# alexandrainst/coral

Measured on AMD Instinct MI355X. Metric: audio-seconds/sec (CTC finetune step: fwd+bwd+allreduce+clip+AdamW), wav2vec2-large, 10 s utterances, higher is better.
Workload: dtype bf16; 1 GPU; wav2vec2-large (XLS-R shape d=1920 L=48 ffn=7680) CTC finetune, 8 x 10 s per GPU, SpecAugment on, activation_dropout 0.1, layerdrop 0 (multi-GPU rule), fp32 master + AdamW + clip 1.0; global_batch=8, frames_per_utt=499, parallelism=dp1

## Files before the change

coral_amd/csrc/ctc.hip:

```cpp
#include "common.h"

#define NEG_INF (-__builtin_inff())

__device__ __forceinline__ float log_add3(float a, float b, float c) {
  const float m = fmaxf(a, fmaxf(b, c));
  if (m == NEG_INF) return NEG_INF;
  return m + __logf(__expf(a - m) + __expf(b - m) + __expf(c - m));
}
__device__ __forceinline__ float log_add2(float a, float b) {
  const float m = fmaxf(a, b);
  if (m == NEG_INF) return NEG_INF;
  return m + __logf(__expf(a - m) + __expf(b - m));
}

struct CtcWs {
  float* lp;
  float* alpha;
  float* beta;
};

__device__ __host__ inline int64_t align256(int64_t x) { return (x + 255) & ~(int64_t)255; }

extern "C" int64_t ca_ctc_workspace_bytes(int32_t B, int32_t T, int32_t Lmax) {
  const int64_t S = 2 * (int64_t)Lmax + 1;
  return align256((int64_t)B * T * 256 * 4) + 2 * align256((int64_t)B * T * S * 4) + align256((int64_t)B * 4);
}

#define CTC_MAXS 1025

__global__ __launch_bounds__(256) void ctc_logsoftmax_kernel(const float* __restrict__ logits, float* __restrict__ lp,
                                                             int64_t frames, int V, int64_t ldv) {
  const int lane = threadIdx.x & 63;
  const int64_t f = (int64_t)blockIdx.x * 4 + (threadIdx.x >> 6);
  if (f >= frames) return;
  const float* l = logits + f * ldv;
  float x[4];
  float mx = NEG_INF;
#pragma unroll
  for (int j = 0; j < 4; ++j) {
    const int v = lane + 64 * j;
    x[j] = v < V ? l[v] : NEG_INF;
    mx = fmaxf(mx, x[j]);
  }
  mx = wave_max(mx);
  float s = 0.f;
#pragma unroll
  for (int j = 0; j < 4; ++j) s += (lane + 64 * j) < V ? __expf(x[j] - mx) : 0.f;
  s = wave_sum(s);
  const float lse = mx + __logf(s);
#pragma unroll
  for (int j = 0; j < 4; ++j)
    if (lane + 64 * j < V) lp[f * V + lane + 64 * j] = x[j] - lse;
}

__global__ __launch_bounds__(512) void ctc_kernel(const int32_t* __restrict__ labels,
                                                  const int32_t* __restrict__ in_len,
                                                  float* __restrict__ nll_out,
                                                  float* __restrict__ raw_nll, const float* __restrict__ lp,
                                                  float* alpha, float* beta, int T, int V,
                                                  int Lmax, int Smax, int blank, int zero_inf, int lp_in_lds) {
  __shared__ int ext[CTC_MAXS];
  __shared__ float rowa[2][CTC_MAXS];
  __shared__ float rowb[2][CTC_MAXS];
  __shared__ int sh_L;
  __shared__ float sh_nll;
  extern __shared__ float lds_lp[];
  const int b = blockIdx.x;
  const int tid = threadIdx.x;
  const int lane = tid & 63, wave = tid >> 6;
  const float* lpb = lp + (int64_t)b * T * V;
  if (lp_in_lds)
    for (int i = tid; i < T * V; i += 512) lds_lp[i] = lpb[i];
  float* ab = alpha + (int64_t)b * T * Smax;
  float* bb = beta + (int64_t)b * T * Smax;
  int Tin = in_len ? in_len[b] : T;
  if (Tin > T) Tin = T;
  if (Tin < 0) Tin = 0;

  if (tid == 0) {
    int L = 0;
    for (int i = 0; i < Lmax; ++i) {
      const int c = labels[(int64_t)b * Lmax + i];
      if (c >= 0) {
        ext[2 * L] = blank;
        ext[2 * L + 1] = c;
        ++L;
      }
    }
    ext[2 * L] = blank;
    sh_L = L;
  }
  __syncthreads();
  const int L = sh_L;
  const int S = 2 * L + 1;
  const bool is_alpha = tid < 256;
  const int st = tid & 255;

  if (S <= 256) {
    if (wave < 2 && Tin > 0) {
      const bool fwd = wave == 0;
      float* tab = fwd ? ab : bb;
      int c[4];
      bool skip[4], valid[4];
      float a[4];
#pragma unroll
      for (int j = 0; j < 4; ++j) {
        const int s = 4 * lane + j;
        valid[j] = s < S;
        c[j] = valid[j] ? ext[s] : blank;
        const int s2 = fwd ? s - 2 : s + 2;
        skip[j] = valid[j] && s2 >= 0 && s2 < S && c[j] != blank && ext[s2] != c[j];
      }
      const int t0 = fwd ? 0 : Tin - 1;
      auto lpv = [&](int tt, int cc) -> float { return lp_in_lds ? lds_lp[tt * V + cc] : lpb[(int64_t)tt * V + cc]; };
#pragma unroll
      for (int j = 0; j < 4; ++j) {
        const int s = 4 * lane + j;
        const bool init = fwd ? (s == 0 || s == 1) : (s == S - 1 || s == S - 2);
        a[j] = (valid[j] && init) ? lpv(t0, c[j]) : NEG_INF;
        if (valid[j]) tab[(int64_t)t0 * Smax + s] = a[j];
      }
      float nx[4];
      if (Tin > 1) {
#pragma unroll
        for (int j = 0; j < 4; ++j) nx[j] = lpv(fwd ? 1 : Tin - 2, c[j]);
      }
      for (int step = 1; step < Tin; ++step) {
        const int tt = fwd ? step : Tin - 1 - step;
        float cur[4];
#pragma unroll
        for (int j = 0; j < 4; ++j) cur[j] = nx[j];
        if (step + 1 < Tin) {
#pragma unroll
          for (int j = 0; j < 4; ++j) nx[j] = lpv(fwd ? step + 1 : Tin - 2 - step, c[j]);
        }
        float n1, n2;
        if (fwd) {
          n1 = __shfl_up(a[3], 1, 64);
          n2 = __shfl_up(a[2], 1, 64);
          if (lane == 0) n1 = n2 = NEG_INF;
        } else {
          n1 = __shfl_down(a[0], 1, 64);
          n2 = __shfl_down(a[1], 1, 64);
          if (lane == 63) n1 = n2 = NEG_INF;
        }
        float na[4];
        if (fwd) {
          na[0] = log_add3(a[0], n1, skip[0] ? n2 : NEG_INF);
          na[1] = log_add3(a[1], a[0], skip[1] ? n1 : NEG_INF);
          na[2] = log_add3(a[2], a[1], skip[2] ? a[0] : NEG_INF);
          na[3] = log_add3(a[3], a[2], skip[3] ? a[1] : NEG_INF);
        } else {
          na[3] = log_add3(a[3], n1, skip[3] ? n2 : NEG_INF);
          na[2] = log_add3(a[2], a[3], skip[2] ? n1 : NEG_INF);
          na[1] = log_add3(a[1], a[2], skip[1] ? a[3] : NEG_INF);
          na[0] = log_add3(a[0], a[1], skip[0] ? a[2] : NEG_INF);
        }
#pragma unroll
        for (int j = 0; j < 4; ++j) {
          a[j] = valid[j] ? na[j] + cur[j] : NEG_INF;
          if (valid[j]) tab[(int64_t)tt * Smax + 4 * lane + j] = a[j];
        }
      }
      if (fwd) {
#pragma unroll
        for (int j = 0; j < 4; ++j)
          if (valid[j]) rowa[(Tin - 1) & 1][4 * lane + j] = a[j];
      }
    }
    __syncthreads();
  } else {
    if (Tin > 0) {
      if (is_alpha) {
        for (int s = st; s < S; s += 256) {
          float a = NEG_INF;
          if (s == 0) a = lpb[blank];
          else if (s == 1) a = lpb[ext[1]];
          rowa[0][s] = a;
          ab[s] = a;
        }
      } else {
        const float* lpt = lpb + (int64_t)(Tin - 1) * V;
        for (int s = st; s < S; s += 256) {
          float v = NEG_INF;
          if (s == S - 1) v = lpt[blank];
          else if (s == S - 2) v = lpt[ext[S - 2]];
          rowb[0][s] = v;
          bb[(int64_t)(Tin - 1) * Smax + s] = v;
        }
      }
    }
    __syncthreads();
    for (int step = 1; step < Tin; ++step) {
      const int cur = step & 1, prv = cur ^ 1;
      if (is_alpha) {
        const int t = step;
        const float* lpt = lpb + (int64_t)t * V;
        for (int s = st; s < S; s += 256) {
          const int c = ext[s];
          const float a0 = rowa[prv][s];
          const float a1 = s >= 1 ? rowa[prv][s - 1] : NEG_INF;
          const float a2 = (s >= 2 && c != blank && ext[s - 2] != c) ? rowa[prv][s - 2] : NEG_INF;
          const float a = log_add3(a0, a1, a2) + lpt[c];
          rowa[cur][s] = a;
          ab[(int64_t)t * Smax + s] = a;
        }
      } else {
        const int t = Tin - 1 - step;
        const float* lpt = lpb + (int64_t)t * V;
        for (int s = st; s < S; s += 256) {
          const int c = ext[s];
          const float b0 = rowb[prv][s];
          const float b1 = s + 1 < S ? rowb[prv][s + 1] : NEG_INF;
          const float b2 =
              (s + 2 < S && c != blank && ext[s + 2] != c) ? rowb[prv][s + 2] : NEG_INF;
          const float v = log_add3(b0, b1, b2) + lpt[c];
          rowb[cur][s] = v;
          bb[(int64_t)t * Smax + s] = v;
        }
      }
      __syncthreads();
    }
  }
  if (tid == 0) {
    float nll;
    if (Tin <= 0) {
      nll = __builtin_inff();
    } else {
      const int lastrow = (Tin - 1) & 1;
      const float l1 = rowa[lastrow][S - 1];
      const float l2 = S >= 2 ? rowa[lastrow][S - 2] : NEG_INF;
      nll = -log_add2(l1, l2);
    }
    sh_nll = nll;
  }
  __syncthreads();
  float nll = sh_nll;
  const bool infeasible = !(nll < __builtin_inff());
  if (tid == 0) {
    nll_out[b] = (infeasible && zero_inf) ? 0.f : nll;
    raw_nll[b] = nll;
  }
}

__global__ __launch_bounds__(512) void ctc_grad_kernel(const int32_t* __restrict__ labels,
                                                       const int32_t* __restrict__ in_len,
                                                       const float* __restrict__ raw_nll, float* __restrict__ grad,
                                                       const float* __restrict__ gscale, const float* __restrict__ lp,
                                                       const float* __restrict__ alpha, const float* __restrict__ beta,
                                                       int T, int V, int64_t ldv, int Lmax, int Smax, int blank) {
  __shared__ int ext[CTC_MAXS];
  __shared__ float vm[8][256], vs[8][256];
  __shared__ int sh_L;
  const int b = blockIdx.y;
  const int tid = threadIdx.x;
  const int lane = tid & 63, wave = tid >> 6;
  if (tid == 0) {
    int L = 0;
    for (int i = 0; i < Lmax; ++i) {
      const int c = labels[(int64_t)b * Lmax + i];
      if (c >= 0) {
        ext[2 * L] = blank;
        ext[2 * L + 1] = c;
        ++L;
      }
    }
    ext[2 * L] = blank;
    sh_L = L;
  }
  __syncthreads();
  const int S = 2 * sh_L + 1;
  int Tin = in_len ? in_len[b] : T;
  if (Tin > T) Tin = T;
  if (Tin < 0) Tin = 0;
  const float nll = raw_nll[b];
  const bool infeasible = !(nll < __builtin_inff());
  const float gs = gscale ? gscale[b] : 1.f;
  const int t = blockIdx.x * 8 + wave;
  if (t >= T) return;
  float* g = grad + ((int64_t)b * T + t) * ldv;
  if (t >= Tin || infeasible) {
    for (int v = lane; v < (int)ldv; v += 64) g[v] = 0.f;
    return;
  }
  float* vmax = vm[wave];
  float* vsum = vs[wave];
  for (int v = lane; v < V; v += 64) {
    vmax[v] = NEG_INF;
    vsum[v] = 0.f;
  }
  const float* at = alpha + ((int64_t)b * T + t) * Smax;
  const float* bt = beta + ((int64_t)b * T + t) * Smax;
  for (int s = lane; s < S; s += 64) {
    const float val = at[s] + bt[s];
    if (val > NEG_INF)
      __builtin_amdgcn_ds_fmaxf((__attribute__((address_space(3))) float*)&vmax[ext[s]], val, 0, 0, false);
  }
  asm volatile("s_waitcnt lgkmcnt(0)" ::: "memory");
  for (int s = lane; s < S; s += 64) {
    const float val = at[s] + bt[s];
    if (val > NEG_INF) {
      const int cc = ext[s];
      __builtin_amdgcn_ds_faddf((__attribute__((address_space(3))) float*)&vsum[cc], __expf(val - vmax[cc]), 0, 0, false);
    }
  }
  asm volatile("s_waitcnt lgkmcnt(0)" ::: "memory");
  const float* lpt = lp + ((int64_t)b * T + t) * V;
  for (int v = lane; v < (int)ldv; v += 64) {
    if (v < V) {
      const float l = lpt[v];
      const float res = vsum[v] > 0.f ? vmax[v] + __logf(vsum[v]) : NEG_INF;
      g[v] = (__expf(l) - __expf(res + nll - l)) * gs;
    } else {
      g[v] = 0.f;
    }
  }
}

extern "C" int ca_ctc_loss_fwd_bwd(const float* logits, const int32_t* labels,
                                   const int32_t* in_len, float* nll, float* grad,
                                   const float* gscale, void* ws, int32_t B, int32_t T, int32_t V,
                                   int64_t ldv, int32_t Lmax, int32_t blank, int32_t zero_infinity,
                                   void* stream) {
  CA_CHECK_ARG(logits && labels && nll && ws, "ca_ctc_loss_fwd_bwd: null pointer");
  CA_CHECK_ARG(B > 0 && T > 0 && V > 0 && V <= 256 && ldv >= V && Lmax >= 0,
               "ca_ctc_loss_fwd_bwd: bad shape (V must be <= 256)");
  CA_CHECK_ARG(2 * Lmax + 1 <= CTC_MAXS, "ca_ctc_loss_fwd_bwd: Lmax %d too long (max %d)", Lmax,
               (CTC_MAXS - 1) / 2);
  CA_CHECK_ARG(blank >= 0 && blank < V, "ca_ctc_loss_fwd_bwd: bad blank");
  const int Smax = 2 * Lmax + 1;
  char* w = (char*)ws;
  float* lp = (float*)w;
  w += align256((int64_t)B * T * 256 * 4);
  float* alpha = (float*)w;
  w += align256((int64_t)B * T * Smax * 4);
  float* beta = (float*)w;
  w += align256((int64_t)B * T * Smax * 4);
  float* raw_nll = (float*)w;
  hipStream_t s = (hipStream_t)stream;
  const int64_t frames = (int64_t)B * T;
  hipLaunchKernelGGL(ctc_logsoftmax_kernel, dim3((unsigned)((frames + 3) / 4)), dim3(256), 0, s, logits, lp, frames, V,
                     ldv);
  const size_t lp_bytes = (size_t)T * V * sizeof(float);
  const int lp_in_lds = lp_bytes <= 120 * 1024 ? 1 : 0;
  static bool attr = false;
  if (!attr) {
    hipFuncSetAttribute((const void*)ctc_kernel, hipFuncAttributeMaxDynamicSharedMemorySize, 120 * 1024);
    attr = true;
  }
  hipLaunchKernelGGL(ctc_kernel, dim3(B), dim3(512), lp_in_lds ? lp_bytes : 0, s, labels, in_len, nll, raw_nll, lp, alpha,
                     beta, T, V, Lmax, Smax, blank, zero_infinity, lp_in_lds);
  if (grad)
    hipLaunchKernelGGL(ctc_grad_kernel, dim3((unsigned)((T + 7) / 8), B), dim3(512), 0, s, labels, in_len, raw_nll, grad,
                       gscale, lp, alpha, beta, T, V, ldv, Lmax, Smax, blank);
  CA_CHECK_LAUNCH("ca_ctc_loss_fwd_bwd");
  return CA_OK;
}

__global__ __launch_bounds__(1024) void ctc_greedy_kernel(const float* __restrict__ logits,
                                                          const int32_t* __restrict__ in_len,
                                                          int32_t* __restrict__ raw,
                                                          int32_t* __restrict__ ids,
                                                          int32_t* __restrict__ out_len, int T,
                                                          int V, int64_t ldv, int blank) {
  extern __shared__ int sh[];
  const int b = blockIdx.x;
  const float* lg = logits + (int64_t)b * T * ldv;
  int32_t* rb = raw + (int64_t)b * T;
  int32_t* ib = ids + (int64_t)b * T;
  int Tin = in_len ? in_len[b] : T;
  if (Tin > T) Tin = T;
  for (int t = threadIdx.x; t < T; t += 1024) {
    const float* l = lg + (int64_t)t * ldv;
    float best = l[0];
    int bi = 0;
    for (int v = 1; v < V; ++v) {
      const float x = l[v];
      if (x > best) {
        best = x;
        bi = v;
      }
    }
    rb[t] = bi;
    ib[t] = -1;
  }
  __syncthreads();
  for (int t = threadIdx.x; t < T; t += 1024) {
    const int c = rb[t];
    sh[t] = (t < Tin && c != blank && (t == 0 || rb[t - 1] != c)) ? 1 : 0;
  }
  __syncthreads();
  for (int off = 1; off < T; off <<= 1) {
    int vals[4];
    int n = 0;
    for (int t = threadIdx.x; t < T; t += 1024) vals[n++] = sh[t] + (t >= off ? sh[t - off] : 0);
    __syncthreads();
    n = 0;
    for (int t = threadIdx.x; t < T; t += 1024) sh[t] = vals[n++];
    __syncthreads();
  }
  for (int t = threadIdx.x; t < T; t += 1024) {
    const int incl = sh[t];
    const int prev = t > 0 ? sh[t - 1] : 0;
    if (incl != prev) ib[incl - 1] = rb[t];
  }
  if (threadIdx.x == 0) out_len[b] = T > 0 ? sh[T - 1] : 0;
}

extern "C" int ca_ctc_greedy_decode(const float* logits, const int32_t* in_len, int32_t* raw,
                                    int32_t* ids, int32_t* out_len, int32_t B, int32_t T,
                                    int32_t V, int64_t ldv, int32_t blank, void* stream) {
  CA_CHECK_ARG(logits && raw && ids && out_len, "ca_ctc_greedy_decode: null pointer");
  CA_CHECK_ARG(B > 0 && T > 0 && T <= 4096 && V > 0 && ldv >= V,
               "ca_ctc_greedy_decode: bad shape (T <= 4096)");
  hipLaunchKernelGGL(ctc_greedy_kernel, dim3(B), dim3(1024), (size_t)T * sizeof(int),
                     (hipStream_t)stream, logits, in_len, raw, ids, out_len, T, V, ldv, blank);
  CA_CHECK_LAUNCH("ca_ctc_greedy_decode");
  return CA_OK;
}
```

coral_amd/csrc/misc.hip:

```cpp
#include "common.h"
#include <cstdlib>

__global__ __launch_bounds__(256) void mask_frames_kernel(unsigned short* __restrict__ h,
                                                          const uint8_t* __restrict__ tmask,
                                                          const uint8_t* __restrict__ fmask,
                                                          const unsigned short* __restrict__ embed,
                                                          const int32_t* __restrict__ flen, int B,
                                                          int T, int C) {
  const int cch = C >> 3;
  const int64_t total = (int64_t)B * T * cch;
  for (int64_t i = (int64_t)blockIdx.x * 256 + threadIdx.x; i < total;
       i += (int64_t)gridDim.x * 256) {
    const int c8 = (int)(i % cch);
    const int64_t bt = i / cch;
    const int t = (int)(bt % T), b = (int)(bt / T);
    const bool tm = tmask && tmask[bt];
    const bool pad = flen && t >= flen[b];
    bool anyf = false;
    if (fmask) {
#pragma unroll
      for (int e = 0; e < 8; ++e) anyf |= fmask[(int64_t)b * C + c8 * 8 + e] != 0;
    }
    if (!tm && !pad && !anyf) continue;
    unsigned short* p = h + bt * C + c8 * 8;
    u16x8_t v = *(u16x8_t*)p;
    if (tm) v = *(const u16x8_t*)(embed + c8 * 8);
    if (fmask) {
#pragma unroll
      for (int e = 0; e < 8; ++e)
        if (fmask[(int64_t)b * C + c8 * 8 + e]) v[e] = 0;
    }
    if (pad) v = (u16x8_t){0, 0, 0, 0, 0, 0, 0, 0};
    *(u16x8_t*)p = v;
  }
}

extern "C" int ca_mask_frames(void* h, const uint8_t* tmask, const uint8_t* fmask,
                              const void* embed, const int32_t* flen, int32_t B, int32_t T,
                              int32_t C, void* stream) {
  CA_CHECK_ARG(h && B > 0 && T > 0 && C > 0 && (C % 8) == 0, "ca_mask_frames: bad argument");
  CA_CHECK_ARG(!tmask || embed, "ca_mask_frames: tmask needs embed");
  int64_t g = ((int64_t)B * T * (C / 8) + 255) / 256;
  if (g > 8192) g = 8192;
  hipLaunchKernelGGL(mask_frames_kernel, dim3((int)g), dim3(256), 0, (hipStream_t)stream,
                     (unsigned short*)h, tmask, fmask, (const unsigned short*)embed, flen, B, T, C);
  CA_CHECK_LAUNCH("ca_mask_frames");
  return CA_OK;
}

__global__ __launch_bounds__(256) void regroup_pad_kernel(const unsigned short* __restrict__ x,
                                                          unsigned short* __restrict__ xg, int B,
                                                          int T, int G, int Cg, int pad) {
  const int cch = Cg >> 3;
  const int Tp = T + 2 * pad;
  const int64_t total = (int64_t)B * G * Tp * cch;
  for (int64_t i = (int64_t)blockIdx.x * 256 + threadIdx.x; i < total;
       i += (int64_t)gridDim.x * 256) {
    const int c8 = (int)(i % cch);
    int64_t r = i / cch;
    const int tp = (int)(r % Tp);
    r /= Tp;
    const int g = (int)(r % G), b = (int)(r / G);
    const int t = tp - pad;
    u16x8_t v = {0, 0, 0, 0, 0, 0, 0, 0};
    if (t >= 0 && t < T) v = *(const u16x8_t*)(x + ((int64_t)b * T + t) * (G * Cg) + g * Cg + c8 * 8);
    *(u16x8_t*)(xg + i * 8) = v;
  }
}

extern "C" int ca_regroup_pad(const void* x, void* xg, int32_t B, int32_t T, int32_t G,
                              int32_t Cg, int32_t pad, void* stream) {
  CA_CHECK_ARG(x && xg && B > 0 && T > 0 && G > 0 && Cg > 0 && (Cg % 8) == 0 && pad >= 0,
               "ca_regroup_pad: bad argument");
  int64_t g = ((int64_t)B * G * (T + 2 * pad) * (Cg / 8) + 255) / 256;
  if (g > 8192) g = 8192;
  hipLaunchKernelGGL(regroup_pad_kernel, dim3((int)g), dim3(256), 0, (hipStream_t)stream,
                     (const unsigned short*)x, (unsigned short*)xg, B, T, G, Cg, pad);
  CA_CHECK_LAUNCH("ca_regroup_pad");
  return CA_OK;
}

#define PCW_SLABS 1024
__global__ __launch_bounds__(256) void tap_dot_kernel(const float* __restrict__ a,
                                                      const float* __restrict__ b,
                                                      float* __restrict__ partial, int64_t nrows,
                                                      int K, int bmode, int Cg, int G) {
  const int j = threadIdx.x % K;
  const int rl = threadIdx.x / K;
  const int nrl = 256 / K;
  const int64_t per = (nrows + gridDim.x - 1) / gridDim.x;
  const int64_t r0 = (int64_t)blockIdx.x * per;
  int64_t r1 = r0 + per;
  if (r1 > nrows) r1 = nrows;
  auto term = [&](int64_t r) -> float {
    const float av = a[r * K + j];
    float bv;
    if (bmode == 0) {
      bv = b[r * K + j];
    } else {
      const int ci = (int)(r % Cg);
      const int64_t co_g = r / Cg;
      bv = b[(co_g * K + j) * Cg + ci];
    }
    return av * bv;
  };
  float acc0 = 0.f, acc1 = 0.f, acc2 = 0.f, acc3 = 0.f;
  int64_t r = r0 + rl;
  for (; r + 3 * nrl < r1; r += 4 * nrl) {
    acc0 += term(r);
    acc1 += term(r + nrl);
    acc2 += term(r + 2 * nrl);
    acc3 += term(r + 3 * nrl);
  }
  for (; r < r1; r += nrl) acc0 += term(r);
  const float acc = (acc0 + acc1) + (acc2 + acc3);
  __shared__ float red[256];
  red[threadIdx.x] = acc;
  __syncthreads();
  if (rl == 0) {
    float t = 0.f;
    for (int q = 0; q < nrl; ++q) t += red[q * K + j];
    partial[(int64_t)blockIdx.x * K + j] = t;
  }
}

__global__ __launch_bounds__(256) void tap_finish_kernel(const float* __restrict__ partial, int nparts, int K,
                                                         float* __restrict__ out, int do_sqrt) {
  __shared__ float red[16][17];
  const int tl = threadIdx.x & 15, pl = threadIdx.x >> 4;
  const int j = blockIdx.x * 16 + tl;
  float a0 = 0.f, a1 = 0.f, a2 = 0.f, a3 = 0.f;
  if (j < K) {
    int p = pl;
    for (; p + 48 < nparts; p += 64) {
      a0 += partial[(int64_t)p * K + j];
      a1 += partial[(int64_t)(p + 16) * K + j];
      a2 += partial[(int64_t)(p + 32) * K + j];
      a3 += partial[(int64_t)(p + 48) * K + j];
    }
    for (; p < nparts; p += 16) a0 += partial[(int64_t)p * K + j];
  }
  red[pl][tl] = (a0 + a1) + (a2 + a3);
  __syncthreads();
  if (pl == 0 && j < K) {
    float t = 0.f;
#pragma unroll
    for (int q = 0; q < 16; ++q) t += red[q][tl];
    out[j] = do_sqrt ? sqrtf(t) : t;
  }
}

__global__ __launch_bounds__(256) void posconv_build_kernel(const float* __restrict__ v,
                                                            const float* __restrict__ gvec,
                                                            const float* __restrict__ norm,
                                                            unsigned short* __restrict__ out,
                                                            int Cg, int K, int mode) {
  extern __shared__ float tile[];
  const int blk = blockIdx.x;
  const float* src;
  int64_t rstride;
  if (mode == 0) {
    src = v + (int64_t)blk * Cg * K;
    rstride = K;
  } else {
    const int g = blk / Cg, ci = blk % Cg;
    src = v + ((int64_t)g * Cg * Cg + ci) * K;
    rstride = (int64_t)Cg * K;
  }
  for (int i = threadIdx.x; i < Cg * K; i += 256) {
    const int r = i / K, j = i % K;
    tile[r * (K + 1) + j] = src[r * rstride + j] * (gvec[j] / norm[j]);
  }
  __syncthreads();
  unsigned short* dst = out + (int64_t)blk * K * Cg;
  for (int i = threadIdx.x; i < Cg * K; i += 256) {
    const int jo = i / Cg, r = i % Cg;
    const int j = mode == 0 ? jo : (K - 1 - jo);
    dst[i] = f2bf(tile[r * (K + 1) + j]);
  }
}

extern "C" int ca_posconv_weight(const float* v, const float* g, void* wf, void* wb, float* norm,
                                 float* partial, int32_t d, int32_t Cg, int32_t K, void* stream) {
  CA_CHECK_ARG(v && g && wf && norm && partial, "ca_posconv_weight: null pointer");
  CA_CHECK_ARG(d > 0 && Cg > 0 && (d % Cg) == 0 && K > 0 && K <= 256 && (256 % K) == 0,
               "ca_posconv_weight: K must divide 256");
  hipStream_t s = (hipStream_t)stream;
  const int64_t nrows = (int64_t)d * Cg;
  hipLaunchKernelGGL(tap_dot_kernel, dim3(PCW_SLABS), dim3(256), 0, s, v, v, partial, nrows, K, 0,
                     Cg, d / Cg);
  hipLaunchKernelGGL(tap_finish_kernel, dim3((K + 15) / 16), dim3(256), 0, s, partial, PCW_SLABS, K, norm, 1);
  const size_t lds = (size_t)Cg * (K + 1) * sizeof(float);
  hipLaunchKernelGGL(posconv_build_kernel, dim3(d), dim3(256), lds, s, v, g, norm,
                     (unsigned short*)wf, Cg, K, 0);
  if (wb)
    hipLaunchKernelGGL(posconv_build_kernel, dim3(d), dim3(256), lds, s, v, g, norm,
                       (unsigned short*)wb, Cg, K, 1);
  CA_CHECK_LAUNCH("ca_posconv_weight");
  return CA_OK;
}

__global__ __launch_bounds__(256) void posconv_wbwd_kernel(const float* __restrict__ dwf,
                                                           const float* __restrict__ v,
                                                           const float* __restrict__ gvec,
                                                           const float* __restrict__ norm,
                                                           const float* __restrict__ dot,
                                                           float* __restrict__ dv, int Cg, int K) {
  extern __shared__ float tile[];
  const int co_g = blockIdx.x;
  const float* src = dwf + (int64_t)co_g * K * Cg;
  for (int i = threadIdx.x; i < K * Cg; i += 256) {
    const int j = i / Cg, ci = i % Cg;
    tile[j * (Cg + 1) + ci] = src[i];
  }
  __syncthreads();
  for (int i = threadIdx.x; i < Cg * K; i += 256) {
    const int ci = i / K, j = i % K;
    const float n = norm[j];
    const int64_t idx = ((int64_t)co_g * Cg + ci) * K + j;
    dv[idx] += (gvec[j] / n) * (tile[j * (Cg + 1) + ci] - v[idx] * dot[j] / (n * n));
  }
}
__global__ void posconv_dg_kernel(const float* __restrict__ dot, const float* __restrict__ norm,
                                  float* __restrict__ dg, int K) {
  const int j = blockIdx.x * blockDim.x + threadIdx.x;
  if (j < K) dg[j] += dot[j] / norm[j];
}

extern "C" int ca_posconv_weight_bwd(const float* dwf, const float* v, const float* g,
                                     const float* norm, float* dv, float* dg, float* partial,
                                     int32_t d, int32_t Cg, int32_t K, void* stream) {
  CA_CHECK_ARG(dwf && v && g && norm && dv && dg && partial, "ca_posconv_weight_bwd: null pointer");
  CA_CHECK_ARG(K > 0 && K <= 256 && (256 % K) == 0, "ca_posconv_weight_bwd: K must divide 256");
  hipStream_t s = (hipStream_t)stream;
  const int64_t nrows = (int64_t)d * Cg;
  float* dot = partial + (int64_t)PCW_SLABS * K;
  hipLaunchKernelGGL(tap_dot_kernel, dim3(PCW_SLABS), dim3(256), 0, s, v, dwf, partial, nrows, K,
                     1, Cg, d / Cg);
  hipLaunchKernelGGL(tap_finish_kernel, dim3((K + 15) / 16), dim3(256), 0, s, partial, PCW_SLABS, K, dot, 0);
  const size_t lds = (size_t)K * (Cg + 1) * sizeof(float);
  hipLaunchKernelGGL(posconv_wbwd_kernel, dim3(d), dim3(256), lds, s, dwf, v, g, norm, dot, dv,
                     Cg, K);
  hipLaunchKernelGGL(posconv_dg_kernel, dim3(1), dim3(256), 0, s, dot, norm, dg, K);
  CA_CHECK_LAUNCH("ca_posconv_weight_bwd");
  return CA_OK;
}

extern "C" int64_t ca_posconv_partial_floats(int32_t K) { return (int64_t)(PCW_SLABS + 1) * K; }

__global__ void cast_f32_bf16_kernel(const float* __restrict__ x, unsigned short* __restrict__ y,
                                     int64_t n) {
  const int64_t n4 = n >> 2;
  for (int64_t i = (int64_t)blockIdx.x * blockDim.x + threadIdx.x; i < n4;
       i += (int64_t)gridDim.x * blockDim.x) {
    const f32x4_t v = *(const f32x4_t*)(x + i * 4);
    *(u16x4_t*)(y + i * 4) = (u16x4_t){f2bf(v[0]), f2bf(v[1]), f2bf(v[2]), f2bf(v[3])};
  }
  if (blockIdx.x == 0 && threadIdx.x < (n & 3)) {
    const int64_t i = (n4 << 2) + threadIdx.x;
    y[i] = f2bf(x[i]);
  }
}
__global__ void cast_bf16_f32_kernel(const unsigned short* __restrict__ x, float* __restrict__ y,
                                     int64_t n) {
  for (int64_t i = (int64_t)blockIdx.x * blockDim.x + threadIdx.x; i < n;
       i += (int64_t)gridDim.x * blockDim.x)
    y[i] = bf2f(x[i]);
}
static int ew_grid(int64_t n, int per) {
  int64_t g = (n / per + 255) / 256;
  if (g > 8192) g = 8192;
  if (g < 1) g = 1;
  return (int)g;
}
extern "C" int ca_cast_f32_bf16(const float* x, void* y, int64_t n, void* stream) {
  CA_CHECK_ARG(x && y && n > 0, "ca_cast_f32_bf16: bad argument");
  CA_CHECK_ARG(((uintptr_t)x % 16) == 0 && ((uintptr_t)y % 8) == 0, "ca_cast_f32_bf16: alignment");
  hipLaunchKernelGGL(cast_f32_bf16_kernel, dim3(ew_grid(n, 4)), dim3(256), 0, (hipStream_t)stream,
                     x, (unsigned short*)y, n);
  CA_CHECK_LAUNCH("ca_cast_f32_bf16");
  return CA_OK;
}
extern "C" int ca_cast_bf16_f32(const void* x, float* y, int64_t n, void* stream) {
  CA_CHECK_ARG(x && y && n > 0, "ca_cast_bf16_f32: bad argument");
  hipLaunchKernelGGL(cast_bf16_f32_kernel, dim3(ew_grid(n, 1)), dim3(256), 0, (hipStream_t)stream,
                     (const unsigned short*)x, y, n);
  CA_CHECK_LAUNCH("ca_cast_bf16_f32");
  return CA_OK;
}

template <bool PACK>
__global__ __launch_bounds__(256) void pack_rows_kernel(const uint4* __restrict__ x, uint4* __restrict__ y,
                                                        const int32_t* __restrict__ row_off, int64_t total, int T, int CPR) {
  const int64_t i = (int64_t)blockIdx.x * 256 + threadIdx.x;
  if (i >= total) return;
  const int64_t row = i / CPR;
  const int ch = (int)(i - row * CPR);
  const int b = (int)(row / T), t = (int)(row - (int64_t)b * T);
  const int r0 = row_off[b];
  int len = row_off[b + 1] - r0;
  len = len < T ? len : T;
  const int64_t j = (int64_t)(r0 + t) * CPR + ch;
  if (PACK) {
    if (t < len) y[j] = x[i];
  } else {
    y[i] = t < len ? x[j] : make_uint4(0u, 0u, 0u, 0u);
  }
}
static int pack_rows_launch(bool pack, const void* x, void* y, const int32_t* row_off, int32_t B, int32_t T, int32_t C,
                            int32_t elt_bytes, void* stream, const char* who) {
  CA_CHECK_ARG(x && y && row_off && x != y && B > 0 && T > 0 && C > 0, "%s: bad argument", who);
  CA_CHECK_ARG(elt_bytes == 2 || elt_bytes == 4, "%s: rows of bf16 (2) or fp32 (4) elements", who);
  const int64_t row_bytes = (int64_t)C * elt_bytes;
  CA_CHECK_ARG((row_bytes % 16) == 0 && ((uintptr_t)x % 16) == 0 && ((uintptr_t)y % 16) == 0,
               "%s: rows must be multiples of 16 bytes, 16-byte aligned", who);
  const int cpr = (int)(row_bytes / 16);
  const int64_t total = (int64_t)B * T * cpr;
  const dim3 grid((unsigned)((total + 255) / 256));
  if (pack)
    hipLaunchKernelGGL(pack_rows_kernel<true>, grid, dim3(256), 0, (hipStream_t)stream, (const uint4*)x, (uint4*)y, row_off,
                       total, T, cpr);
  else
    hipLaunchKernelGGL(pack_rows_kernel<false>, grid, dim3(256), 0, (hipStream_t)stream, (const uint4*)x, (uint4*)y, row_off,
                       total, T, cpr);
  CA_CHECK_LAUNCH(who);
  return CA_OK;
}
extern "C" int ca_pack_rows(const void* x, void* y, const int32_t* row_off, int32_t B, int32_t T, int32_t C,
                            int32_t elt_bytes, void* stream) {
  return pack_rows_launch(true, x, y, row_off, B, T, C, elt_bytes, stream, "ca_pack_rows");
}
extern "C" int ca_unpack_rows(const void* x, void* y, const int32_t* row_off, int32_t B, int32_t T, int32_t C,
                              int32_t elt_bytes, void* stream) {
  return pack_rows_launch(false, x, y, row_off, B, T, C, elt_bytes, stream, "ca_unpack_rows");
}

__global__ __launch_bounds__(256) void transpose_f32_bf16_kernel(const float* __restrict__ x,
                                                                 unsigned short* __restrict__ y,
                                                                 int rows, int cols) {
  __shared__ float tile[32][33];
  const int c0 = blockIdx.x * 32, r0 = blockIdx.y * 32;
  const int tx = threadIdx.x & 31, ty = threadIdx.x >> 5;
  for (int k = ty; k < 32; k += 8) {
    const int r = r0 + k, c = c0 + tx;
    tile[k][tx] = (r < rows && c < cols) ? x[(int64_t)r * cols + c] : 0.f;
  }
  __syncthreads();
  for (int k = ty; k < 32; k += 8) {
    const int c = c0 + k, r = r0 + tx;
    if (c < cols && r < rows) y[(int64_t)c * rows + r] = f2bf(tile[tx][k]);
  }
}
extern "C" int ca_transpose_f32_bf16(const float* x, void* y, int32_t rows, int32_t cols,
                                     void* stream) {
  CA_CHECK_ARG(x && y && rows > 0 && cols > 0, "ca_transpose_f32_bf16: bad argument");
  hipLaunchKernelGGL(transpose_f32_bf16_kernel, dim3((cols + 31) / 32, (rows + 31) / 32),
                     dim3(256), 0, (hipStream_t)stream, x, (unsigned short*)y, rows, cols);
  CA_CHECK_LAUNCH("ca_transpose_f32_bf16");
  return CA_OK;
}

__global__ void conv_w_reorder_kernel(const float* __restrict__ w, unsigned short* __restrict__ wr,
                                      int64_t n, int Ci, int k) {
  for (int64_t i = (int64_t)blockIdx.x * blockDim.x + threadIdx.x; i < n;
       i += (int64_t)gridDim.x * blockDim.x) {
    const int ci = (int)(i % Ci);
    const int64_t r = i / Ci;
    const int j = (int)(r % k);
    const int64_t co = r / k;
    wr[i] = f2bf(w[(co * Ci + ci) * k + j]);
  }
}
extern "C" int ca_conv_weight_reorder(const float* w, void* wr, int32_t Co, int32_t Ci, int32_t k,
                                      void* stream) {
  CA_CHECK_ARG(w && wr && Co > 0 && Ci > 0 && k > 0, "ca_conv_weight_reorder: bad argument");
  const int64_t n = (int64_t)Co * Ci * k;
  hipLaunchKernelGGL(conv_w_reorder_kernel, dim3(ew_grid(n, 1)), dim3(256), 0,
                     (hipStream_t)stream, w, (unsigned short*)wr, n, Ci, k);
  CA_CHECK_LAUNCH("ca_conv_weight_reorder");
  return CA_OK;
}
__global__ void conv_w_grad_reorder_kernel(const float* __restrict__ dwr, float* __restrict__ dw,
                                           int64_t n, int Ci, int k) {
  for (int64_t i = (int64_t)blockIdx.x * blockDim.x + threadIdx.x; i < n;
       i += (int64_t)gridDim.x * blockDim.x) {
    const int ci = (int)(i % Ci);
    const int64_t r = i / Ci;
    const int j = (int)(r % k);
    const int64_t co = r / k;
    dw[(co * Ci + ci) * k + j] += dwr[i];
  }
}
extern "C" int ca_conv_weight_grad_reorder(const float* dwr, float* dw, int32_t Co, int32_t Ci,
                                           int32_t k, void* stream) {
  CA_CHECK_ARG(dwr && dw && Co > 0 && Ci > 0 && k > 0, "ca_conv_weight_grad_reorder: bad arg");
  const int64_t n = (int64_t)Co * Ci * k;
// ... 318 lines not shown
```

Measured before the change: 1125 audio-seconds/sec.

## Speed up CTC recursion with log2 math/DPP and retile pos-conv weight backward

The CTC alpha/beta wave pass moves to base-2 log-sum-exp using hardware exp2/log and DPP lane shifts. Skip checks are limited to odd states, the LDS log-prob copy is pre-scaled by log2(e), and loads are prefetched two rows ahead. Separately, the positional-conv weight-norm backward is rebuilt as a tiled dot kernel and a vectorised dv kernel with nontemporal loads and stores, and the dg update is folded into the finish kernel, which drops one launch. Both target small serial or latency-bound kernels, so their effect on the whole finetune step should be small. The base-2 conversion adds some rounding differences.

```diff
diff --git a/coral_amd/csrc/ctc.hip b/coral_amd/csrc/ctc.hip
--- a/coral_amd/csrc/ctc.hip
+++ b/coral_amd/csrc/ctc.hip
@@ -53,12 +53,106 @@
     if (lane + 64 * j < V) lp[f * V + lane + 64 * j] = x[j] - lse;
 }
 
+#define CTC_LOG2E 1.4426950408889634f
+#define CTC_LN2 0.6931471805599453f
+template <bool FWD> __device__ __forceinline__ float ctc_neighbour(float v) {
+  return __builtin_bit_cast(float, __builtin_amdgcn_update_dpp(__builtin_bit_cast(int, NEG_INF), __builtin_bit_cast(int, v),
+                                                               FWD ? 0x138 : 0x130, 0xf, 0xf, false));
+}
+__device__ __forceinline__ float log2_add2(float a, float b) {
+  const float m = fmaxf(a, b), lo = fminf(a, b);
+  const float ms = fmaxf(m, -1e30f);
+  return m + __builtin_amdgcn_logf(1.0f + __builtin_amdgcn_exp2f(lo - ms));
+}
+__device__ __forceinline__ float log2_add3(float a, float b, float c) {
+  const float m = fmaxf(a, fmaxf(b, c)), lo = fminf(a, fminf(b, c)), md = __builtin_amdgcn_fmed3f(a, b, c);
+  const float ms = fmaxf(m, -1e30f);
+  return m + __builtin_amdgcn_logf(1.0f + __builtin_amdgcn_exp2f(md - ms) + __builtin_amdgcn_exp2f(lo - ms));
+}
+
+template <bool FWD, bool LP_LDS>
+__device__ __forceinline__ void ctc_wave_pass(const int* ext, const float* lp2, const float* __restrict__ lpb,
+                                              float* __restrict__ tab, int lane, int S, int Tin, int V, int Smax, int blank,
+                                              float (&last)[4]) {
+  int c[4];
+  bool valid[4], skip[4];
+  float dead[4];
+#pragma unroll
+  for (int j = 0; j < 4; ++j) {
+    const int s = 4 * lane + j;
+    valid[j] = s < S;
+    c[j] = valid[j] ? ext[s] : blank;
+    const int s2 = FWD ? s - 2 : s + 2;
+    skip[j] = (j & 1) && valid[j] && s2 >= 0 && s2 < S && c[j] != blank && ext[s2] != c[j];
+    dead[j] = valid[j] ? 0.f : NEG_INF;
+  }
+  auto emit = [&](int tt, int j) -> float {
+    if (LP_LDS) return lp2[tt * V + c[j]] + dead[j];
+    return fmaf(lpb[(int64_t)tt * V + c[j]], CTC_LOG2E, dead[j]);
+  };
+  auto row = [&](int step) -> int {
+    const int t = FWD ? step : Tin - 1 - step;
+    return t < 0 ? 0 : (t > Tin - 1 ? Tin - 1 : t);
+  };
+  const int t0 = row(0);
+  float a[4];
+#pragma unroll
+  for (int j = 0; j < 4; ++j) {
+    const int s = 4 * lane + j;
+    const bool init = FWD ? (s == 0 || s == 1) : (s == S - 1 || s == S - 2);
+    last[j] = (valid[j] && init) ? lpb[(int64_t)t0 * V + c[j]] : NEG_INF;
+    a[j] = last[j] * CTC_LOG2E;
+    if (valid[j]) tab[(int64_t)t0 * Smax + s] = last[j];
+  }
+  float nx1[4], nx2[4];
+#pragma unroll
+  for (int j = 0; j < 4; ++j) {
+    nx1[j] = emit(row(1), j);
+    nx2[j] = emit(row(2), j);
+  }
+  for (int step = 1; step < Tin; ++step) {
+    float cur[4];
+    const int t2 = row(step + 2);
+#pragma unroll
+    for (int j = 0; j < 4; ++j) {
+      cur[j] = nx1[j];
+      nx1[j] = nx2[j];
+      nx2[j] = emit(t2, j);
+    }
+    float na[4];
+    if (FWD) {
+      const float n1 = ctc_neighbour<true>(a[3]);
+      na[0] = log2_add2(a[0], n1);
+      na[1] = log2_add3(a[1], a[0], skip[1] ? n1 : NEG_INF);
+      na[2] = log2_add2(a[2], a[1]);
+      na[3] = log2_add3(a[3], a[2], skip[3] ? a[1] : NEG_INF);
+    } else {
+      const float n1 = ctc_neighbour<false>(a[0]);
+      const float n2 = ctc_neighbour<false>(a[1]);
+      na[3] = log2_add3(a[3], n1, skip[3] ? n2 : NEG_INF);
+      na[2] = log2_add2(a[2], a[3]);
+      na[1] = log2_add3(a[1], a[2], skip[1] ? a[3] : NEG_INF);
+      na[0] = log2_add2(a[0], a[1]);
+    }
+    float* trow = tab + (int64_t)row(step) * Smax + 4 * lane;
+#pragma unroll
+    for (int j = 0; j < 4; ++j) {
+      a[j] = na[j] + cur[j];
+      last[j] = a[j] * CTC_LN2;
+    }
+#pragma unroll
+    for (int j = 0; j < 4; ++j)
+      if (valid[j]) trow[j] = last[j];
+  }
+}
+
+template <bool LP_LDS>
 __global__ __launch_bounds__(512) void ctc_kernel(const int32_t* __restrict__ labels,
                                                   const int32_t* __restrict__ in_len,
                                                   float* __restrict__ nll_out,
                                                   float* __restrict__ raw_nll, const float* __restrict__ lp,
                                                   float* alpha, float* beta, int T, int V,
-                                                  int Lmax, int Smax, int blank, int zero_inf, int lp_in_lds) {
+                                                  int Lmax, int Smax, int blank, int zero_inf) {
   __shared__ int ext[CTC_MAXS];
   __shared__ float rowa[2][CTC_MAXS];
   __shared__ float rowb[2][CTC_MAXS];
@@ -69,8 +163,8 @@
   const int tid = threadIdx.x;
   const int lane = tid & 63, wave = tid >> 6;
   const float* lpb = lp + (int64_t)b * T * V;
-  if (lp_in_lds)
-    for (int i = tid; i < T * V; i += 512) lds_lp[i] = lpb[i];
+  if (LP_LDS)
+    for (int i = tid; i < T * V; i += 512) lds_lp[i] = lpb[i] * CTC_LOG2E;
   float* ab = alpha + (int64_t)b * T * Smax;
   float* bb = beta + (int64_t)b * T * Smax;
   int Tin = in_len ? in_len[b] : T;
@@ -98,74 +192,14 @@
 
   if (S <= 256) {
     if (wave < 2 && Tin > 0) {
-      const bool fwd = wave == 0;
-      float* tab = fwd ? ab : bb;
-      int c[4];
-      bool skip[4], valid[4];
-      float a[4];
-#pragma unroll
-      for (int j = 0; j < 4; ++j) {
-        const int s = 4 * lane + j;
-        valid[j] = s < S;
-        c[j] = valid[j] ? ext[s] : blank;
-        const int s2 = fwd ? s - 2 : s + 2;
-        skip[j] = valid[j] && s2 >= 0 && s2 < S && c[j] != blank && ext[s2] != c[j];
-      }
-      const int t0 = fwd ? 0 : Tin - 1;
-      auto lpv = [&](int tt, int cc) -> float { return lp_in_lds ? lds_lp[tt * V + cc] : lpb[(int64_t)tt * V + cc]; };
-#pragma unroll
-      for (int j = 0; j < 4; ++j) {
-        const int s = 4 * lane + j;
-        const bool init = fwd ? (s == 0 || s == 1) : (s == S - 1 || s == S - 2);
-        a[j] = (valid[j] && init) ? lpv(t0, c[j]) : NEG_INF;
-        if (valid[j]) tab[(int64_t)t0 * Smax + s] = a[j];
-      }
-      float nx[4];
-      if (Tin > 1) {
-#pragma unroll
-        for (int j = 0; j < 4; ++j) nx[j] = lpv(fwd ? 1 : Tin - 2, c[j]);
-      }
-      for (int step = 1; step < Tin; ++step) {
-        const int tt = fwd ? step : Tin - 1 - step;
-        float cur[4];
-#pragma unroll
-        for (int j = 0; j < 4; ++j) cur[j] = nx[j];
-        if (step + 1 < Tin) {
-#pragma unroll
-          for (int j = 0; j < 4; ++j) nx[j] = lpv(fwd ? step + 1 : Tin - 2 - step, c[j]);
-        }
-        float n1, n2;
-        if (fwd) {
-          n1 = __shfl_up(a[3], 1, 64);
-          n2 = __shfl_up(a[2], 1, 64);
-          if (lane == 0) n1 = n2 = NEG_INF;
-        } else {
-          n1 = __shfl_down(a[0], 1, 64);
-          n2 = __shfl_down(a[1], 1, 64);
-          if (lane == 63) n1 = n2 = NEG_INF;
-        }
-        float na[4];
-        if (fwd) {
-          na[0] = log_add3(a[0], n1, skip[0] ? n2 : NEG_INF);
-          na[1] = log_add3(a[1], a[0], skip[1] ? n1 : NEG_INF);
-          na[2] = log_add3(a[2], a[1], skip[2] ? a[0] : NEG_INF);
-          na[3] = log_add3(a[3], a[2], skip[3] ? a[1] : NEG_INF);
-        } else {
-          na[3] = log_add3(a[3], n1, skip[3] ? n2 : NEG_INF);
-          na[2] = log_add3(a[2], a[3], skip[2] ? n1 : NEG_INF);
-          na[1] = log_add3(a[1], a[2], skip[1] ? a[3] : NEG_INF);
-          na[0] = log_add3(a[0], a[1], skip[0] ? a[2] : NEG_INF);
-        }
-#pragma unroll
-        for (int j = 0; j < 4; ++j) {
-          a[j] = valid[j] ? na[j] + cur[j] : NEG_INF;
-          if (valid[j]) tab[(int64_t)tt * Smax + 4 * lane + j] = a[j];
-        }
-      }
-      if (fwd) {
+      float last[4];
+      if (wave == 0) {
+        ctc_wave_pass<true, LP_LDS>(ext, lds_lp, lpb, ab, lane, S, Tin, V, Smax, blank, last);
 #pragma unroll
         for (int j = 0; j < 4; ++j)
-          if (valid[j]) rowa[(Tin - 1) & 1][4 * lane + j] = a[j];
+          if (4 * lane + j < S) rowa[(Tin - 1) & 1][4 * lane + j] = last[j];
+      } else {
+        ctc_wave_pass<false, LP_LDS>(ext, lds_lp, lpb, bb, lane, S, Tin, V, Smax, blank, last);
       }
     }
     __syncthreads();
@@ -345,11 +379,15 @@
   const int lp_in_lds = lp_bytes <= 120 * 1024 ? 1 : 0;
   static bool attr = false;
   if (!attr) {
-    hipFuncSetAttribute((const void*)ctc_kernel, hipFuncAttributeMaxDynamicSharedMemorySize, 120 * 1024);
+    hipFuncSetAttribute((const void*)ctc_kernel<true>, hipFuncAttributeMaxDynamicSharedMemorySize, 120 * 1024);
     attr = true;
   }
-  hipLaunchKernelGGL(ctc_kernel, dim3(B), dim3(512), lp_in_lds ? lp_bytes : 0, s, labels, in_len, nll, raw_nll, lp, alpha,
-                     beta, T, V, Lmax, Smax, blank, zero_infinity, lp_in_lds);
+  if (lp_in_lds)
+    hipLaunchKernelGGL(ctc_kernel<true>, dim3(B), dim3(512), lp_bytes, s, labels, in_len, nll, raw_nll, lp, alpha, beta,
+                       T, V, Lmax, Smax, blank, zero_infinity);
+  else
+    hipLaunchKernelGGL(ctc_kernel<false>, dim3(B), dim3(512), 0, s, labels, in_len, nll, raw_nll, lp, alpha, beta, T, V,
+                       Lmax, Smax, blank, zero_infinity);
   if (grad)
     hipLaunchKernelGGL(ctc_grad_kernel, dim3((unsigned)((T + 7) / 8), B), dim3(512), 0, s, labels, in_len, raw_nll, grad,
                        gscale, lp, alpha, beta, T, V, ldv, Lmax, Smax, blank);
diff --git a/coral_amd/csrc/misc.hip b/coral_amd/csrc/misc.hip
--- a/coral_amd/csrc/misc.hip
+++ b/coral_amd/csrc/misc.hip
@@ -81,6 +81,33 @@
 }
 
 #define PCW_SLABS 1024
+#define PCW_JT 32
+
+template <int W> struct pcw_vec { float e[W]; };
+template <int W, bool NT> __device__ __forceinline__ pcw_vec<W> pcw_load(const float* p) {
+  pcw_vec<W> r;
+  if constexpr (W == 4) {
+    const f32x4_t t = NT ? __builtin_nontemporal_load((const f32x4_t*)p) : *(const f32x4_t*)p;
+    r.e[0] = t[0], r.e[1] = t[1], r.e[2] = t[2], r.e[3] = t[3];
+  } else {
+    r.e[0] = NT ? __builtin_nontemporal_load(p) : *p;
+  }
+  return r;
+}
+template <int W> __device__ __forceinline__ void pcw_store_nt(float* p, const pcw_vec<W>& r) {
+  if constexpr (W == 4)
+    __builtin_nontemporal_store((f32x4_t){r.e[0], r.e[1], r.e[2], r.e[3]}, (f32x4_t*)p);
+  else
+    __builtin_nontemporal_store(r.e[0], p);
+}
+__device__ __forceinline__ void pcw_tree(float* red, int lanes, int width) {
+  for (int s = lanes >> 1; s >= 1; s >>= 1) {
+    __syncthreads();
+    for (int i = threadIdx.x; i < s * width; i += 256) red[i] += red[i + s * width];
+  }
+  __syncthreads();
+}
+
 __global__ __launch_bounds__(256) void tap_dot_kernel(const float* __restrict__ a,
                                                       const float* __restrict__ b,
                                                       float* __restrict__ partial, int64_t nrows,
@@ -125,7 +152,8 @@
 }
 
 __global__ __launch_bounds__(256) void tap_finish_kernel(const float* __restrict__ partial, int nparts, int K,
-                                                         float* __restrict__ out, int do_sqrt) {
+                                                         float* __restrict__ out, int mode,
+                                                         const float* __restrict__ norm, float* __restrict__ dg) {
   __shared__ float red[16][17];
   const int tl = threadIdx.x & 15, pl = threadIdx.x >> 4;
   const int j = blockIdx.x * 16 + tl;
@@ -146,7 +174,12 @@
     float t = 0.f;
 #pragma unroll
     for (int q = 0; q < 16; ++q) t += red[q][tl];
-    out[j] = do_sqrt ? sqrtf(t) : t;
+    if (mode == 0) {
+      out[j] = sqrtf(t);
+    } else {
+      out[j] = t;
+      if (mode == 2) dg[j] += t / norm[j];
+    }
   }
 }
 
@@ -189,7 +222,8 @@
   const int64_t nrows = (int64_t)d * Cg;
   hipLaunchKernelGGL(tap_dot_kernel, dim3(PCW_SLABS), dim3(256), 0, s, v, v, partial, nrows, K, 0,
                      Cg, d / Cg);
-  hipLaunchKernelGGL(tap_finish_kernel, dim3((K + 15) / 16), dim3(256), 0, s, partial, PCW_SLABS, K, norm, 1);
+  hipLaunchKernelGGL(tap_finish_kernel, dim3((K + 15) / 16), dim3(256), 0, s, partial, PCW_SLABS, K, norm, 0,
+                     (const float*)nullptr, (float*)nullptr);
   const size_t lds = (size_t)Cg * (K + 1) * sizeof(float);
   hipLaunchKernelGGL(posconv_build_kernel, dim3(d), dim3(256), lds, s, v, g, norm,
                      (unsigned short*)wf, Cg, K, 0);
@@ -200,31 +234,114 @@
   return CA_OK;
 }
 
-__global__ __launch_bounds__(256) void posconv_wbwd_kernel(const float* __restrict__ dwf,
-                                                           const float* __restrict__ v,
-                                                           const float* __restrict__ gvec,
-                                                           const float* __restrict__ norm,
-                                                           const float* __restrict__ dot,
-                                                           float* __restrict__ dv, int Cg, int K) {
+struct pcw_geom {
+  int JT, nJ, jq, cil, S;
+};
+__host__ __device__ __forceinline__ pcw_geom pcw_geometry(int Cg, int K, int W) {
+  pcw_geom g;
+  g.JT = K < PCW_JT ? K : PCW_JT;
+  g.nJ = K / g.JT;
+  g.jq = g.JT / W;
+  g.cil = 256 / g.jq;
+  g.S = ((Cg + 7) & ~7) + 2;
+  return g;
+}
+template <int W>
+__device__ __forceinline__ void pcw_fill_tile(float* tile, const float* __restrict__ src, int JT, int Cg, int S) {
+  const int n = JT * Cg / W;
+  for (int i0 = threadIdx.x; i0 < n; i0 += 4 * 256) {
+    pcw_vec<W> t[4];
+#pragma unroll
+    for (int q = 0; q < 4; ++q)
+      if (i0 + q * 256 < n) t[q] = pcw_load<W, true>(src + (int64_t)(i0 + q * 256) * W);
+#pragma unroll
+    for (int q = 0; q < 4; ++q)
+      if (i0 + q * 256 < n) {
+        const int e0 = (i0 + q * 256) * W;
+        const int j = e0 / Cg, ci = e0 - j * Cg;
+#pragma unroll
+        for (int e = 0; e < W; ++e) tile[j * S + ci + e] = t[q].e[e];
+      }
+  }
+}
+
+template <int W>
+__global__ __launch_bounds__(256) void posconv_dot_kernel(const float* __restrict__ dwf, const float* __restrict__ v,
+                                                          float* __restrict__ partial, int d, int Cg, int K,
+                                                          int per_co) {
   extern __shared__ float tile[];
-  const int co_g = blockIdx.x;
-  const float* src = dwf + (int64_t)co_g * K * Cg;
-  for (int i = threadIdx.x; i < K * Cg; i += 256) {
-    const int j = i / Cg, ci = i % Cg;
-    tile[j * (Cg + 1) + ci] = src[i];
-  }
+  __shared__ float red[256 * W];
+  const pcw_geom g = pcw_geometry(Cg, K, W);
+  const int slab = blockIdx.x / g.nJ, j0 = (blockIdx.x % g.nJ) * g.JT;
+  const int jl = (threadIdx.x % g.jq) * W, cl = threadIdx.x / g.jq;
+  float acc[W];
+#pragma unroll
+  for (int e = 0; e < W; ++e) acc[e] = 0.f;
+  int co1 = (slab + 1) * per_co;
+  if (co1 > d) co1 = d;
+  for (int co = slab * per_co; co < co1; ++co) {
+    __syncthreads();
+    pcw_fill_tile<W>(tile, dwf + ((int64_t)co * K + j0) * Cg, g.JT, Cg, g.S);
+    __syncthreads();
+    const float* vr = v + (int64_t)co * Cg * K + j0 + jl;
+    for (int c0 = cl; c0 < Cg; c0 += 4 * g.cil) {
+      pcw_vec<W> t[4];
+#pragma unroll
+      for (int q = 0; q < 4; ++q)
+        if (c0 + q * g.cil < Cg) t[q] = pcw_load<W, true>(vr + (int64_t)(c0 + q * g.cil) * K);
+#pragma unroll
+      for (int q = 0; q < 4; ++q)
+        if (c0 + q * g.cil < Cg) {
+#pragma unroll
+          for (int e = 0; e < W; ++e) acc[e] = fmaf(t[q].e[e], tile[(jl + e) * g.S + c0 + q * g.cil], acc[e]);
+        }
+    }
+  }
+#pragma unroll
+  for (int e = 0; e < W; ++e) red[cl * g.JT + jl + e] = acc[e];
+  pcw_tree(red, g.cil, g.JT);
+  if ((int)threadIdx.x < g.JT) partial[(int64_t)slab * K + j0 + threadIdx.x] = red[threadIdx.x];
+}
+
+template <int W>
+__global__ __launch_bounds__(256) void posconv_dv_kernel(const float* __restrict__ dwf, const float* __restrict__ v,
+                                                         const float* __restrict__ gvec,
+                                                         const float* __restrict__ norm,
+                                                         const float* __restrict__ dot, float* __restrict__ dv,
+                                                         int Cg, int K) {
+  extern __shared__ float tile[];
+  const pcw_geom g = pcw_geometry(Cg, K, W);
+  const int co = blockIdx.x / g.nJ, j0 = (blockIdx.x % g.nJ) * g.JT;
+  const int jl = (threadIdx.x % g.jq) * W, cl = threadIdx.x / g.jq;
+  float gn[W], nn[W], dt[W];
+#pragma unroll
+  for (int e = 0; e < W; ++e) {
+    const float n = norm[j0 + jl + e];
+    gn[e] = gvec[j0 + jl + e] / n;
+    nn[e] = n * n;
+    dt[e] = dot[j0 + jl + e];
+  }
+  pcw_fill_tile<W>(tile, dwf + ((int64_t)co * K + j0) * Cg, g.JT, Cg, g.S);
   __syncthreads();
-  for (int i = threadIdx.x; i < Cg * K; i += 256) {
-    const int ci = i / K, j = i % K;
-    const float n = norm[j];
-    const int64_t idx = ((int64_t)co_g * Cg + ci) * K + j;
-    dv[idx] += (gvec[j] / n) * (tile[j * (Cg + 1) + ci] - v[idx] * dot[j] / (n * n));
-  }
-}
-__global__ void posconv_dg_kernel(const float* __restrict__ dot, const float* __restrict__ norm,
-                                  float* __restrict__ dg, int K) {
-  const int j = blockIdx.x * blockDim.x + threadIdx.x;
-  if (j < K) dg[j] += dot[j] / norm[j];
+  const int64_t base = (int64_t)co * Cg * K + j0 + jl;
+  for (int c0 = cl; c0 < Cg; c0 += 4 * g.cil) {
+    pcw_vec<W> tv[4], td[4];
+#pragma unroll
+    for (int q = 0; q < 4; ++q)
+      if (c0 + q * g.cil < Cg) {
+        tv[q] = pcw_load<W, true>(v + base + (int64_t)(c0 + q * g.cil) * K);
+        td[q] = pcw_load<W, true>(dv + base + (int64_t)(c0 + q * g.cil) * K);
+      }
+#pragma unroll
+    for (int q = 0; q < 4; ++q)
+      if (c0 + q * g.cil < Cg) {
+        const int ci = c0 + q * g.cil;
+#pragma unroll
+        for (int e = 0; e < W; ++e)
+          td[q].e[e] += gn[e] * (tile[(jl + e) * g.S + ci] - tv[q].e[e] * dt[e] / nn[e]);
+        pcw_store_nt<W>(dv + base + (int64_t)ci * K, td[q]);
+      }
+  }
 }
 
 extern "C" int ca_posconv_weight_bwd(const float* dwf, const float* v, const float* g,
@@ -232,16 +349,24 @@
                                      int32_t d, int32_t Cg, int32_t K, void* stream) {
   CA_CHECK_ARG(dwf && v && g && norm && dv && dg && partial, "ca_posconv_weight_bwd: null pointer");
   CA_CHECK_ARG(K > 0 && K <= 256 && (256 % K) == 0, "ca_posconv_weight_bwd: K must divide 256");
+  CA_CHECK_ARG(d > 0 && Cg > 0, "ca_posconv_weight_bwd: bad shape");
   hipStream_t s = (hipStream_t)stream;
-  const int64_t nrows = (int64_t)d * Cg;
+  const bool wide = (K & 3) == 0 && (Cg & 3) == 0 && (((uintptr_t)dwf | (uintptr_t)v | (uintptr_t)dv) & 15) == 0;
+  const pcw_geom ge = pcw_geometry(Cg, K, wide ? 4 : 1);
+  const size_t lds = (size_t)ge.JT * ge.S * sizeof(float);
+  CA_CHECK_ARG(lds <= 60 * 1024, "ca_posconv_weight_bwd: Cg = %d does not fit the LDS tile", Cg);
+  const int per_co = (d + PCW_SLABS - 1) / PCW_SLABS;
+  const int nslab = (d + per_co - 1) / per_co;
   float* dot = partial + (int64_t)PCW_SLABS * K;
-  hipLaunchKernelGGL(tap_dot_kernel, dim3(PCW_SLABS), dim3(256), 0, s, v, dwf, partial, nrows, K,
-                     1, Cg, d / Cg);
-  hipLaunchKernelGGL(tap_finish_kernel, dim3((K + 15) / 16), dim3(256), 0, s, partial, PCW_SLABS, K, dot, 0);
-  const size_t lds = (size_t)K * (Cg + 1) * sizeof(float);
-  hipLaunchKernelGGL(posconv_wbwd_kernel, dim3(d), dim3(256), lds, s, dwf, v, g, norm, dot, dv,
-                     Cg, K);
-  hipLaunchKernelGGL(posconv_dg_kernel, dim3(1), dim3(256), 0, s, dot, norm, dg, K);
+  if (wide)
+    hipLaunchKernelGGL(posconv_dot_kernel<4>, dim3(nslab * ge.nJ), dim3(256), lds, s, dwf, v, partial, d, Cg, K, per_co);
+  else
+    hipLaunchKernelGGL(posconv_dot_kernel<1>, dim3(nslab * ge.nJ), dim3(256), lds, s, dwf, v, partial, d, Cg, K, per_co);
+  hipLaunchKernelGGL(tap_finish_kernel, dim3((K + 15) / 16), dim3(256), 0, s, partial, nslab, K, dot, 2, norm, dg);
+  if (wide)
+    hipLaunchKernelGGL(posconv_dv_kernel<4>, dim3(d * ge.nJ), dim3(256), lds, s, dwf, v, g, norm, dot, dv, Cg, K);
+  else
+    hipLaunchKernelGGL(posconv_dv_kernel<1>, dim3(d * ge.nJ), dim3(256), lds, s, dwf, v, g, norm, dot, dv, Cg, K);
   CA_CHECK_LAUNCH("ca_posconv_weight_bwd");
   return CA_OK;
 }
```

Result: no change. 1132 audio-seconds/sec, median of 6 (+0.6%).
